# c0gent/hbbft

Hardware: AMD Instinct MI355X
Metric: verified BLS sig shares/sec (whole node) + combine latency, N=64 f=21 (higher is better)
Workload: dtype u32 limbs (Fp, 14x28-bit); 1 GPU; ThresholdSign share verification, BASELINE configs[1]; batch_per_gpu=65536, streams=2, documents_per_gpu=1024, n_nodes=64, f=21, pairing_impl=auto, parallelism=shard-by-batch x1

## Files before the change

hbbft_amd/csrc/ofp.hpp:

```cpp
#pragma once
#include "qfp.hpp"

namespace hbs {

HP_D int o_idx() { return (int)((threadIdx.x >> 1) & 3); }

HP_D int32_t o_swz4(int32_t v) { return __builtin_amdgcn_ds_swizzle(v, 0x101F); }
HP_D Fp o_swz4_fp(const Fp& a) {
  Fp r;
#pragma unroll
  for (int i = 0; i < NL; i++) r.l[i] = o_swz4(a.l[i]);
  return r;
}

HP_D Fp o_sel(int o, const Fp& a0, const Fp& a1, const Fp& a2, const Fp& a3) {
  const bool b0 = (o & 1) != 0, b1 = (o & 2) != 0;
  Fp r;
#pragma unroll
  for (int i = 0; i < NL; i++) {
    const int32_t lo = b0 ? a1.l[i] : a0.l[i];
    const int32_t hi = b0 ? a3.l[i] : a2.l[i];
    r.l[i] = b1 ? hi : lo;
  }
  return r;
}

HP_D void o_gather(int o, const Fp& mine, Fp (&r)[4]) {
  const Fp m1 = dpp_fp<DPP_QSWAP>(mine);
  const bool b0 = (o & 1) != 0, b1 = (o & 2) != 0;
  Fp e, d;
#pragma unroll
  for (int i = 0; i < NL; i++) {
    e.l[i] = b0 ? m1.l[i] : mine.l[i];
    d.l[i] = b0 ? mine.l[i] : m1.l[i];
  }
  const Fp e2 = o_swz4_fp(e), d2 = o_swz4_fp(d);
#pragma unroll
  for (int i = 0; i < NL; i++) {
    r[0].l[i] = b1 ? e2.l[i] : e.l[i];
    r[1].l[i] = b1 ? d2.l[i] : d.l[i];
    r[2].l[i] = b1 ? e.l[i] : e2.l[i];
    r[3].l[i] = b1 ? d.l[i] : d2.l[i];
  }
}

HP_D void h_mul4(const Fp (&x)[4], const Fp (&y)[4], Fp (&r)[4]) {
  const int o = o_idx();
  o_gather(o, h_mul(o_sel(o, x[0], x[1], x[2], x[3]), o_sel(o, y[0], y[1], y[2], y[3])), r);
}
HP_D void h_sqr4(const Fp (&x)[4], Fp (&r)[4]) {
  const int o = o_idx();
  o_gather(o, h_sqr(o_sel(o, x[0], x[1], x[2], x[3])), r);
}
HP_D void fp_mul4(const Fp (&x)[4], const Fp (&y)[4], Fp (&r)[4]) {
  const int o = o_idx();
  o_gather(o, fp_mul(o_sel(o, x[0], x[1], x[2], x[3]), o_sel(o, y[0], y[1], y[2], y[3])), r);
}

HP_D void h6_mul_pair_o(const H6& a, const H6& b, const H6& c, const H6& d, H6& ab, H6& cd) {
  Fp r[4];
  {
    const Fp x[4] = {a.c1, a.c2, c.c1, c.c2}, y[4] = {b.c1, b.c2, d.c1, d.c2};
    h_mul4(x, y, r);
  }
  const Fp av1 = r[0], av2 = r[1], cv1 = r[2], cv2 = r[3];
  {
    const Fp x[4] = {fp_addl(a.c1, a.c2), a.c0, fp_addl(c.c1, c.c2), c.c0};
    const Fp y[4] = {fp_add(b.c1, b.c2), b.c0, fp_add(d.c1, d.c2), d.c0};
    h_mul4(x, y, r);
  }
  const Fp av0 = r[1], cv0 = r[3];
  ab.c0 = fp_red_l(h_add_xi_l(av0, fp_sub2l(r[0], av1, av2)));
  cd.c0 = fp_red_l(h_add_xi_l(cv0, fp_sub2l(r[2], cv1, cv2)));
  {
    const Fp x[4] = {fp_addl(a.c0, a.c1), fp_addl(a.c0, a.c2), fp_addl(c.c0, c.c1), fp_addl(c.c0, c.c2)};
    const Fp y[4] = {fp_add(b.c0, b.c1), fp_add(b.c0, b.c2), fp_add(d.c0, d.c1), fp_add(d.c0, d.c2)};
    h_mul4(x, y, r);
  }
  ab.c1 = fp_red_l(h_add_xi_l(fp_sub2l(r[0], av0, av1), av2));
  ab.c2 = fp_red_l(fp_addl(fp_sub2l(r[1], av0, av2), av1));
  cd.c1 = fp_red_l(h_add_xi_l(fp_sub2l(r[2], cv0, cv1), cv2));
  cd.c2 = fp_red_l(fp_addl(fp_sub2l(r[3], cv0, cv2), cv1));
}

HP_D H6 h6_mul_o(const H6& a, const H6& b) {
  Fp r[4];
  {
    const Fp x[4] = {a.c1, a.c2, fp_addl(a.c1, a.c2), a.c0};
    const Fp y[4] = {b.c1, b.c2, fp_add(b.c1, b.c2), b.c0};
    h_mul4(x, y, r);
  }
  const Fp v1 = r[0], v2 = r[1], t12 = r[2], v0 = r[3];
  {
    const Fp x[4] = {fp_addl(a.c0, a.c1), fp_addl(a.c0, a.c2), a.c0, a.c0};
    const Fp y[4] = {fp_add(b.c0, b.c1), fp_add(b.c0, b.c2), b.c0, b.c0};
    h_mul4(x, y, r);
  }
  return {fp_red_l(h_add_xi_l(v0, fp_sub2l(t12, v1, v2))), fp_red_l(h_add_xi_l(fp_sub2l(r[0], v0, v1), v2)),
          fp_red_l(fp_addl(fp_sub2l(r[1], v0, v2), v1))};
}

HP_D H12 h12_cyclo_sqr_o(const H12& f) {
  const Fp& a0 = f.c0.c0; const Fp& a2 = f.c0.c1; const Fp& a4 = f.c0.c2;
  const Fp& a1 = f.c1.c0; const Fp& a3 = f.c1.c1; const Fp& a5 = f.c1.c2;
  Fp r1[4], r2[4];
  {
    const Fp x[4] = {a0, a3, a1, a4};
    h_sqr4(x, r1);
  }
  {
    const Fp x[4] = {fp_add(a0, a3), fp_add(a1, a4), a2, a5};
    h_sqr4(x, r2);
  }
  const Fp s25 = h_sqr(fp_add(a2, a5));
  const Fp &s0 = r1[0], &s3 = r1[1], &s1 = r1[2], &s4 = r1[3];
  const Fp &s03 = r2[0], &s14 = r2[1], &s2 = r2[2], &s5 = r2[3];
  H12 r;
  r.c0.c0 = fp_red_mk<3, -2>(h_add_xi_l(s0, s3), a0);
  r.c1.c1 = fp_red_mk<3, 2>(fp_sub2l(s03, s0, s3), a3);
  r.c0.c1 = fp_red_mk<3, -2>(h_add_xi_l(s1, s4), a2);
  r.c1.c2 = fp_red_mk<3, 2>(fp_sub2l(s14, s1, s4), a5);
  r.c0.c2 = fp_red_mk<3, -2>(h_add_xi_l(s2, s5), a4);
  r.c1.c0 = fp_red_mk<3, 2>(h_add_xi_l(fp_zero(), fp_sub2l(s25, s2, s5)), a1);
  return r;
}

HP_D H12 h12_frob1_o(const H12& f) {
  Fp r[4];
  const Fp x[4] = {h_conj(f.c1.c0), h_conj(f.c0.c1), h_conj(f.c1.c1), h_conj(f.c0.c2)};
  const Fp y[4] = {HP_FROB1(1), HP_FROB1(2), HP_FROB1(3), HP_FROB1(4)};
  h_mul4(x, y, r);
  H12 o;
  o.c0.c0 = h_conj(f.c0.c0);
  o.c1.c0 = r[0];
  o.c0.c1 = r[1];
  o.c1.c1 = r[2];
  o.c0.c2 = r[3];
  o.c1.c2 = h_mul(h_conj(f.c1.c2), HP_FROB1(5));
  return h12_red(o);
}
HP_D H12 h12_frob2_o(const H12& f) {
  Fp r[4];
  const Fp x[4] = {f.c1.c0, f.c0.c1, f.c1.c1, f.c0.c2};
  const Fp y[4] = {fp_const(hb::FROB2_1_C0), fp_const(hb::FROB2_2_C0), fp_const(hb::FROB2_3_C0),
                   fp_const(hb::FROB2_4_C0)};
  fp_mul4(x, y, r);
  H12 o;
  o.c0.c0 = f.c0.c0;
  o.c1.c0 = r[0];
  o.c0.c1 = r[1];
  o.c1.c1 = r[2];
  o.c0.c2 = r[3];
  o.c1.c2 = fp_mul(f.c1.c2, fp_const(hb::FROB2_5_C0));
  return o;
}

HP_D HLine h_dbl_step_o(HJac& T) {
  Fp r[4];
  {
    const Fp x[4] = {T.x, T.y, T.z, fp_add(T.y, T.z)};
    h_sqr4(x, r);
  }
  const Fp A = r[0], B = r[1], ZZ = r[2], YZ = r[3];
  const Fp E = fp_lin(3, A, 0, A);
  {
    const Fp xb = fp_add(T.x, B);
    const Fp x[4] = {B, xb, E, E}, y[4] = {B, xb, E, T.x};
    h_mul4(x, y, r);
  }
  const Fp C = r[0], XB = r[1], F = r[2], EX = r[3];
  const Fp D = fp_lin(2, fp_sub(fp_sub(XB, A), C), 0, C);
  const Fp Z3 = fp_sub(fp_sub(YZ, B), ZZ);
  const Fp X3 = fp_sub(F, fp_add(D, D));
  {
    const Fp x[4] = {E, Z3, E, E}, y[4] = {ZZ, ZZ, fp_sub(D, X3), ZZ};
    h_mul4(x, y, r);
  }
  HLine l;
  l.c0 = fp_reduce(fp_sub(EX, fp_add(B, B)));
  l.c1 = fp_neg(r[0]);
  l.c4 = r[1];
  T.y = fp_reduce(fp_sub(r[2], fp_lin(8, C, 0, C)));
  T.x = fp_reduce(X3);
  T.z = fp_reduce(Z3);
  return l;
}

HP_D HLine h_add_step_o(HJac& T, const Fp& xQ, const Fp& yQ) {
  Fp r[4];
  {
    const Fp x[4] = {T.z, yQ, T.z, T.z}, y[4] = {T.z, T.z, T.z, T.z};
    h_mul4(x, y, r);
  }
  const Fp Z1Z1 = r[0], YZ = r[1];
  {
    const Fp x[4] = {xQ, YZ, xQ, xQ}, y[4] = {Z1Z1, Z1Z1, Z1Z1, Z1Z1};
    h_mul4(x, y, r);
  }
  const Fp H = fp_sub(r[0], T.x);
  const Fp rr = fp_sub(r[1], T.y);
  {
    const Fp x[4] = {H, rr, T.z, H}, y[4] = {H, rr, H, H};
    h_mul4(x, y, r);
  }
  const Fp HH = r[0], R2 = r[1], Z3 = r[2];
  {
    const Fp x[4] = {H, T.x, yQ, rr}, y[4] = {HH, HH, Z3, xQ};
    h_mul4(x, y, r);
  }
  const Fp HHH = r[0], V = r[1], YZ3 = r[2], RX = r[3];
  const Fp X3 = fp_sub(fp_sub(R2, HHH), fp_add(V, V));
  {
    const Fp x[4] = {rr, T.y, rr, rr}, y[4] = {fp_sub(V, X3), HHH, fp_sub(V, X3), fp_sub(V, X3)};
    h_mul4(x, y, r);
  }
  HLine l;
  l.c0 = fp_reduce(fp_sub(RX, YZ3));
  l.c1 = fp_neg(rr);
  l.c4 = Z3;
  T.x = fp_reduce(X3);
  T.y = fp_reduce(fp_sub(r[0], r[1]));
  T.z = Z3;
  return l;
}

struct LaneOcto {
  static constexpr int LANES = 8;
  static HP_D bool leader() { return (threadIdx.x & 7) == 0; }
  static HP_D bool value_writer() { return o_idx() == 0; }
  using Walk = HJac;
  static HP_D HLine dbl_step(HJac& T) { return h_dbl_step_o(T); }
  static HP_D HLine add_step(HJac& T, const Fp& xQ, const Fp& yQ) { return h_add_step_o(T, xQ, yQ); }

  static HP_D H6 mul6(const H6& a, const H6& b) { return h6_mul_o(a, b); }
  template <class A1, class B1>
  static HP_D void mul6x2(const H6& a0, const H6& b0, const A1& a1, const B1& b1, H6& r0, H6& r1) {
    h6_mul_pair_o(a0, b0, h6_of(a1), h6_of(b1), r0, r1);
  }
  static HP_D void mul6x2_12(const H6& a0, const H6& b0, const H6& a1, const Fp& c1, const Fp& c2, H6& r0, H6& r1) {
    h6_mul_pair_o(a0, b0, a1, {h_zero(), c1, c2}, r0, r1);
  }
  static HP_D void line_product(const Fp& a0, const Fp& a1, const Fp& a4, const Fp& b0, const Fp& b1, const Fp& b4,
                                H6& C0, Fp& c11, Fp& c12) {
    Fp r[4];
    {
      const Fp x[4] = {a0, a1, a4, fp_addl(a0, a4)}, y[4] = {b0, b1, b4, fp_add(b0, b4)};
      h_mul4(x, y, r);
    }
    const Fp a0b0 = r[0], a1b1 = r[1], a4b4 = r[2], t04 = r[3];
    {
      const Fp x[4] = {fp_addl(a1, a4), fp_addl(a0, a1), a0, a0}, y[4] = {fp_add(b1, b4), fp_add(b0, b1), b0, b0};
      h_mul4(x, y, r);
    }
    h_line_comb(a0b0, a1b1, a4b4, t04, r[0], r[1], C0, c11, c12);
  }
  static HP_D H12 cyclo_sqr(const H12& f) { return h12_cyclo_sqr_o(f); }
  static HP_D H12 frob1(const H12& f) { return h12_frob1_o(f); }
  static HP_D H12 frob2(const H12& f) { return h12_frob2_o(f); }

  template <bool G1, bool G2, class RA, class RB, class ST>
  static HP_D void lines_at_p(const RA& raw_a, const RB& raw_b, const ST& A, const ST& B, bool neg2, HLine& la,
                              HLine& lb) {
    const HLine ra = raw_a();
    const HLine rb = raw_b();
    Fp r[4];
    const Fp x[4] = {ra.c1, ra.c4, rb.c1, rb.c4};
    const Fp y[4] = {side_xP<G1>(A), side_yP<G1>(A, false), side_xP<G2>(B), side_yP<G2>(B, neg2)};
    fp_mul4(x, y, r);
    la.c0 = A.act ? ra.c0 : h_one();
    la.c1 = A.act ? r[0] : fp_zero();
    la.c4 = A.act ? r[1] : fp_zero();
    lb.c0 = B.act ? rb.c0 : h_one();
    lb.c1 = B.act ? r[2] : fp_zero();
    lb.c4 = B.act ? r[3] : fp_zero();
  }
};

}
```

hbbft_amd/csrc/pair_side.hpp:

```cpp
#pragma once
#include "launch.hpp"
#include "qfp.hpp"

namespace hbs {

constexpr int PAIR_STEPS = 68;
constexpr int PL_Q4 = 11;
constexpr int STASH_WORDS = 72;

HP_D void stash_fp(uint32_t* __restrict__ s, const Fp& a) {
  const Fp r = fp_reduce(a);
  Fp rp = fp_addl(r, fp_const(P_L));
  fp_norm(rp);
  const Fp c = (r.l[NL - 1] < 0) ? rp : r;
#pragma unroll
  for (int w = 0; w < 12; w++) {
    const int bit = 32 * w, li = bit / 28, sh = bit % 28;
    uint64_t v = (uint64_t)(uint32_t)c.l[li] >> sh;
    if (li + 1 < NL) v |= (uint64_t)(uint32_t)c.l[li + 1] << (28 - sh);
    if (li + 2 < NL) v |= (uint64_t)(uint32_t)c.l[li + 2] << (56 - sh);
    s[w * 256] = (uint32_t)v;
  }
}
HP_D Fp unstash_fp(const uint32_t* __restrict__ s) {
  uint32_t w[12];
#pragma unroll
  for (int k = 0; k < 12; k++) w[k] = s[k * 256];
  Fp r;
#pragma unroll
  for (int i = 0; i < NL; i++) {
    const int bit = 28 * i, wi = bit >> 5, sh = bit & 31;
    uint64_t v = w[wi];
    if (wi + 1 < 12) v |= (uint64_t)w[wi + 1] << 32;
    r.l[i] = (int32_t)((uint32_t)(v >> sh) & (uint32_t)MASK28);
  }
  return r;
}
HP_D void stash12(uint32_t* __restrict__ s, const H12& f) {
  stash_fp(s + 0 * 12 * 256, f.c0.c0);
  stash_fp(s + 1 * 12 * 256, f.c0.c1);
  stash_fp(s + 2 * 12 * 256, f.c0.c2);
  stash_fp(s + 3 * 12 * 256, f.c1.c0);
  stash_fp(s + 4 * 12 * 256, f.c1.c1);
  stash_fp(s + 5 * 12 * 256, f.c1.c2);
}
HP_D H12 unstash12(const uint32_t* __restrict__ s) {
  H12 f;
  f.c0.c0 = unstash_fp(s + 0 * 12 * 256);
  f.c0.c1 = unstash_fp(s + 1 * 12 * 256);
  f.c0.c2 = unstash_fp(s + 2 * 12 * 256);
  f.c1.c0 = unstash_fp(s + 3 * 12 * 256);
  f.c1.c1 = unstash_fp(s + 4 * 12 * 256);
  f.c1.c2 = unstash_fp(s + 5 * 12 * 256);
  return f;
}

struct PairSide {
  const uint32_t* p;
  const uint32_t* q;
  const int4* lines;
  const uint8_t* qinf;
  const uint32_t* idx;
  uint32_t nq;
};

template <class ST>
HP_D void side_q(const PairSide& s, const ST& st, Fp& xQ, Fp& yQ) {
  h_g2_load(s.q + (size_t)st.q * 48, xQ, yQ);
  if (st.qinf) {
    xQ = h_one();
    yQ = h_one();
  }
}

template <bool WALK, bool GEN, class ST>
HP_D bool side_init(const PairSide& s, int i, bool negate, ST& st) {
  st.q = s.idx ? s.idx[i] : (uint32_t)i;
  if (st.q >= s.nq) return false;
  bool pinf;
  if (GEN) {
    pinf = false;
  } else if (s.p) {
    const uint32_t* w = s.p + (size_t)i * 24;
    pinf = words_zero(w, 24);
    st.xP = fp_from_words(w);
    st.yP = fp_from_words(w + 12);
  } else {
    pinf = false;
    st.xP = fp_const(hb::G1X_M);
    st.yP = fp_const(hb::G1Y_M);
  }
  if (!GEN && negate) st.yP = fp_neg(st.yP);
  if (WALK) {
    const uint32_t* w = s.q + (size_t)st.q * 48;
    st.qinf = lp_both(words_zero(w + (lp_even() ? 0 : 12), 12) && words_zero(w + (lp_even() ? 24 : 36), 12));
    Fp xQ, yQ;
    side_q(s, st, xQ, yQ);
    st.T = {xQ, yQ, h_one()};
  } else {
    st.qinf = s.qinf[st.q] != 0;
  }
  st.act = !pinf && !st.qinf;
  return true;
}

constexpr int LINE_Q4 = 2 * PL_Q4;
HP_D size_t line_at(size_t e) { return e * LINE_Q4 + (lp_even() ? 0 : PL_Q4); }
HP_D HLine line_load(const int4* __restrict__ p) {
  int32_t w[4 * PL_Q4];
#pragma unroll
  for (int k = 0; k < PL_Q4; k++) {
    const int4 v = p[k];
    w[4 * k] = v.x; w[4 * k + 1] = v.y; w[4 * k + 2] = v.z; w[4 * k + 3] = v.w;
  }
  HLine l;
#pragma unroll
  for (int j = 0; j < NL; j++) {
    l.c0.l[j] = w[j];
    l.c1.l[j] = w[NL + j];
    l.c4.l[j] = w[2 * NL + j];
  }
  return l;
}
HP_D void line_store(int4* __restrict__ p, const HLine& l) {
  int32_t w[4 * PL_Q4];
#pragma unroll
  for (int j = 0; j < NL; j++) {
    w[j] = l.c0.l[j];
    w[NL + j] = l.c1.l[j];
    w[2 * NL + j] = l.c4.l[j];
  }
  w[3 * NL] = 0;
  w[3 * NL + 1] = 0;
#pragma unroll
  for (int k = 0; k < PL_Q4; k++) p[k] = make_int4(w[4 * k], w[4 * k + 1], w[4 * k + 2], w[4 * k + 3]);
}

template <class G, bool WALK, bool DBL, class ST>
HP_D HLine side_raw(const PairSide& s, ST& st, int step) {
  if constexpr (!WALK) {
    return line_load(s.lines + line_at(st.q * PAIR_STEPS + step));
  } else if constexpr (DBL) {
    return G::dbl_step(st.T);
  } else {
    Fp xQ, yQ;
    side_q(s, st, xQ, yQ);
    return G::add_step(st.T, xQ, yQ);
  }
}

struct PairArgs {
  int n;
  PairSide s1, s2;
  int flags;
  uint8_t* verdict;
  uint32_t* value_out;
};


template <class G, bool PLUS1>
HP_D H12 exp_abs_x_gs(const H12& base) {
  const uint64_t e = PLUS1 ? hb::X_ABS + 1 : hb::X_ABS;
  H12 r = base;
#pragma unroll 1
  for (int k = 62; k >= 0; k--) {
    r = G::cyclo_sqr(r);
    if ((e >> k) & 1) r = h12_mul<G>(r, base);
  }
  return r;
}
template <class G>
struct ExpGs {
  HP_D H12 x(const H12& f) { return h12_conj(exp_abs_x_gs<G, false>(f)); }
  HP_D H12 xm1(const H12& f) { return h12_conj(exp_abs_x_gs<G, true>(f)); }
};

template <class G, class Exp>
HP_D H12 final_exp(const H12& f, uint32_t* __restrict__ stash) {
  const H12 f1 = h12_mul<G>(h12_conj(f), h12_inv<G>(f));
  const H12 g = h12_mul<G>(G::frob2(f1), f1);
  stash12(stash, g);
  Exp ex;
  H12 a = ex.xm1(ex.xm1(g));
  const H12 b = h12_mul<G>(ex.x(a), G::frob1(a));
  {
    const H12 gs = unstash12(stash);
    const H12 w = h12_mul<G>(h12_mul<G>(G::frob2(b), h12_conj(b)), h12_mul<G>(G::cyclo_sqr(gs), gs));
    stash12(stash, w);
  }
  const H12 c = ex.x(ex.x(b));
  return h12_mul<G>(c, unstash12(stash));
}

template <class G, class Exp, bool W1, bool W2, int GEN>
HP_D void lane_verify(const PairArgs& a, uint32_t* stash) {
  const int i = (int)((blockIdx.x * 256u + threadIdx.x) / (unsigned)G::LANES);
  if (i >= a.n) return;
  constexpr bool G1 = GEN == 1, G2 = GEN == 2;
  const bool neg2 = (a.flags & 1) != 0;
  SideStateT<typename G::Walk> A, B;
  const bool ok1 = side_init<W1, G1>(a.s1, i, false, A);
  const bool ok2 = side_init<W2, G2>(a.s2, i, neg2, B);
  if (!ok1 || !ok2) {
    if (G::leader() && a.verdict) a.verdict[i] = 0;
    return;
  }
  H12 f = h12_one();
  int step = 0;
#pragma unroll 1
  for (int b = 62; b >= 0; b--) {
    if (b != 62) f = h12_sqr<G>(f);
    {
      HLine la, lb;
      G::template lines_at_p<G1, G2>([&]() HP_L { return side_raw<G, W1, true>(a.s1, A, step); },
                                     [&]() HP_L { return side_raw<G, W2, true>(a.s2, B, step); }, A, B, neg2, la, lb);
      f = h12_mul_lines<G>(f, la.c0, la.c1, la.c4, lb.c0, lb.c1, lb.c4);
    }
    step++;
    if ((hb::X_ABS >> b) & 1) {
      HLine la, lb;
      G::template lines_at_p<G1, G2>([&]() HP_L { return side_raw<G, W1, false>(a.s1, A, step); },
                                     [&]() HP_L { return side_raw<G, W2, false>(a.s2, B, step); }, A, B, neg2, la, lb);
      f = h12_mul_lines<G>(f, la.c0, la.c1, la.c4, lb.c0, lb.c1, lb.c4);
      step++;
    }
  }
  if (a.flags & 2) f = h12_conj(f);
  const H12 e = final_exp<G, Exp>(f, stash + threadIdx.x);
  if (a.value_out && G::value_writer()) {
    uint32_t* o = a.value_out + (size_t)i * 144 + (lp_even() ? 0 : 12);
    fp_to_words(e.c0.c0, o + 0);
    fp_to_words(e.c0.c1, o + 24);
    fp_to_words(e.c0.c2, o + 48);
    fp_to_words(e.c1.c0, o + 72);
    fp_to_words(e.c1.c1, o + 96);
    fp_to_words(e.c1.c2, o + 120);
  }
  const bool one = h12_is_one(e);
  if (G::leader() && a.verdict) a.verdict[i] = one ? 1 : 0;
}

}

namespace hbl {

inline hbs::PairArgs pair_args(int n, const PairSideDesc& d1, const PairSideDesc& d2, int flags, uint8_t* verdict,
                               uint32_t* value_out) {
  hbs::PairArgs a;
  a.n = n;
  const PairSideDesc* d[2] = {&d1, &d2};
  hbs::PairSide* o[2] = {&a.s1, &a.s2};
  for (int k = 0; k < 2; k++) {
    o[k]->p = (const uint32_t*)d[k]->p;
    o[k]->q = (const uint32_t*)d[k]->q;
    o[k]->lines = (const int4*)d[k]->lines;
    o[k]->qinf = d[k]->qinf;
    o[k]->idx = d[k]->idx;
    o[k]->nq = (uint32_t)d[k]->nq;
  }
  a.flags = flags;
  a.verdict = verdict;
  a.value_out = value_out;
  return a;
}

inline int pair_gen_mode(const PairSideDesc& d1, const PairSideDesc& d2) {
  return (d1.p == nullptr) == (d2.p == nullptr) ? 0 : (d1.p == nullptr ? 1 : 2);
}

template <class K, int GEN>
hipError_t lane_launch(hipStream_t s, int n, const PairSideDesc& d1, const PairSideDesc& d2, int flags,
                       uint8_t* verdict, uint32_t* value_out) {
  const hbs::PairArgs a = pair_args(n, d1, d2, flags, verdict, value_out);
  const dim3 grid((unsigned)((K::LANES * (size_t)n + 255) / 256)), block(256);
  const size_t lds = (size_t)hbs::STASH_WORDS * 256 * 4;
  const bool w1 = d1.lines == nullptr, w2 = d2.lines == nullptr;
  if (w1 && w2)
    hipLaunchKernelGGL((K::template kernel<true, true, GEN>), grid, block, lds, s, a);
  else if (w1)
    hipLaunchKernelGGL((K::template kernel<true, false, GEN>), grid, block, lds, s, a);
  else if (w2)
    hipLaunchKernelGGL((K::template kernel<false, true, GEN>), grid, block, lds, s, a);
  else
    hipLaunchKernelGGL((K::template kernel<false, false, GEN>), grid, block, lds, s, a);
  return hipGetLastError();
}

}
```

hbbft_amd/csrc/pfp.hpp:

```cpp
#pragma once
#include "sfp.hpp"
#include "words.hpp"

#ifndef HP_INV_MODE
#define HP_INV_MODE 0
#endif

#define HP_D __device__ __forceinline__
#define HP_L __attribute__((always_inline))

namespace hbs {

constexpr int DPP_SWAP = 0xB1;
constexpr int DPP_EVEN = 0xA0;
constexpr int DPP_ODD = 0xF5;

HP_D bool lp_even() { return (threadIdx.x & 1) == 0; }
template <int CTRL>
HP_D int32_t dpp(int32_t v) {
  return __builtin_amdgcn_mov_dpp(v, CTRL, 0xF, 0xF, true);
}
template <int CTRL>
HP_D Fp dpp_fp(const Fp& a) {
  Fp r;
// ... 168 lines not shown
  const bool one = (ev ? part_one : mine_one) != 0;
  uint32_t v[N + 1];
#pragma unroll
  for (int i = 0; i <= N; i++) {
    const uint32_t pv = (uint32_t)dpp<DPP_SWAP>((int32_t)co[i]);
    v[i] = ev ? pv : co[i];
  }
  hb::words_reduce_32m<N>(v, mod);
#pragma unroll
  for (int i = 0; i < N; i++) out[i] = one ? v[i] : 0u;
}

template <int MODE = 0>
HP_D Fp h_inv_vartime(const Fp& a) {
  const Fp s = fp_sqr(a);
  const Fp n = fp_add(s, dpp_fp<DPP_SWAP>(s));
  uint32_t w[12], p[12], r[12];
  fp_to_words(n, w);
  uint32_t nz = 0;
#pragma unroll
  for (int i = 0; i < 12; i++) nz |= w[i];
  if (nz == 0) return fp_zero();
#pragma unroll
  for (int i = 0; i < 12; i++) p[i] = hb::PM2_W[i];
  p[0] += 2;
  if ((MODE & INV_PAIR) != 0)
    lp_inv_uniform<12>(w, p, r);
  else
    hb::words_inv_vartime<12, MODE>(w, p, r);
  return h_conj(fp_mul(a, fp_from_words(r)));
}

template <int M, int K>
HP_D Fp fp_red_mk(const Fp& t, const Fp& a) {
  const int64_t top = (int64_t)t.l[NL - 1] * M + (int64_t)K * a.l[NL - 1];
  const int32_t q = (int32_t)((top * QINV) >> 32);
  Fp r;
  int64_t acc = 0;
#pragma unroll
  for (int i = 0; i < NL - 1; i++) {
    acc += (int64_t)t.l[i] * M + (int64_t)K * a.l[i] - (int64_t)q * (int32_t)P_L[i];
    r.l[i] = (int32_t)acc & MASK28;
    acc >>= 28;
  }
  r.l[NL - 1] = (int32_t)(acc + top - (int64_t)q * (int32_t)P_L[NL - 1]);
  return r;
}
HP_D Fp fp_red_l(const Fp& t) { return fp_red_mk<1, 0>(t, t); }
HP_D Fp h_add_xi_l(const Fp& s, const Fp& t) {
  const int32_t sm = lp_even() ? -1 : 0;
  const Fp pt = dpp_fp<DPP_SWAP>(t);
  Fp r;
#pragma unroll
  for (int i = 0; i < NL; i++) r.l[i] = s.l[i] + t.l[i] + ((pt.l[i] ^ sm) - sm);
  return r;
}
HP_D Fp fp_sub2l(const Fp& a, const Fp& b, const Fp& c) {
  Fp r;
#pragma unroll
  for (int i = 0; i < NL; i++) r.l[i] = a.l[i] - b.l[i] - c.l[i];
  return r;
}

HP_D Fp h_xi_l(const Fp& t) {
  const int32_t sm = lp_even() ? -1 : 0;
  const Fp pt = dpp_fp<DPP_SWAP>(t);
  Fp r;
#pragma unroll
  for (int i = 0; i < NL; i++) r.l[i] = t.l[i] + ((pt.l[i] ^ sm) - sm);
  return r;
}

struct H6 { Fp c0, c1, c2; };
struct H12 { H6 c0, c1; };

HP_D H6 h6_zero() { return {h_zero(), h_zero(), h_zero()}; }
HP_D H6 h6_one() { return {h_one(), h_zero(), h_zero()}; }
HP_D H6 h6_add(const H6& a, const H6& b) { return {fp_add(a.c0, b.c0), fp_add(a.c1, b.c1), fp_add(a.c2, b.c2)}; }
HP_D H6 h6_sub(const H6& a, const H6& b) { return {fp_sub(a.c0, b.c0), fp_sub(a.c1, b.c1), fp_sub(a.c2, b.c2)}; }
HP_D H6 h6_neg(const H6& a) { return {fp_neg(a.c0), fp_neg(a.c1), fp_neg(a.c2)}; }
HP_D H6 h6_red(const H6& a) { return {fp_reduce(a.c0), fp_reduce(a.c1), fp_reduce(a.c2)}; }
HP_D H6 h6_mul_v(const H6& a) { return {h_mul_xi(a.c2), a.c0, a.c1}; }

HP_D H6 h6_mul(const H6& a, const H6& b) {
  const Fp v1 = h_mul(a.c1, b.c1);
  const Fp v2 = h_mul(a.c2, b.c2);
  const Fp d0 = fp_sub2l(h_mul(fp_addl(a.c1, a.c2), fp_add(b.c1, b.c2)), v1, v2);
  const Fp v0 = h_mul(a.c0, b.c0);
  const Fp c0 = fp_red_l(h_add_xi_l(v0, d0));
  const Fp c1 = fp_red_l(h_add_xi_l(fp_sub2l(h_mul(fp_addl(a.c0, a.c1), fp_add(b.c0, b.c1)), v0, v1), v2));
  const Fp c2 = fp_red_l(fp_addl(fp_sub2l(h_mul(fp_addl(a.c0, a.c2), fp_add(b.c0, b.c2)), v0, v2), v1));
  return {c0, c1, c2};
}
HP_D H6 h6_inv(const H6& a) {
  const Fp c0 = fp_reduce(fp_sub(h_sqr(a.c0), h_mul_xi(h_mul(a.c1, a.c2))));
  const Fp c1 = fp_reduce(fp_sub(h_mul_xi(h_sqr(a.c2)), h_mul(a.c0, a.c1)));
  const Fp c2 = fp_reduce(fp_sub(h_sqr(a.c1), h_mul(a.c0, a.c2)));
  const Fp t = fp_reduce(fp_add(h_mul(a.c0, c0), h_mul_xi(fp_add(h_mul(a.c2, c1), h_mul(a.c1, c2)))));
  const Fp ti = fp_reduce(h_inv_vartime<HP_INV_MODE>(t));
  return {h_mul(c0, ti), h_mul(c1, ti), h_mul(c2, ti)};
}

HP_D H12 h12_one() { return {h6_one(), h6_zero()}; }
HP_D H12 h12_conj(const H12& a) { return {a.c0, h6_neg(a.c1)}; }
HP_D H12 h12_red(const H12& a) { return {h6_red(a.c0), h6_red(a.c1)}; }
HP_D H12 h12_kcomb(const H6& t0, const H6& t1, const H6& s) {
  return {{fp_red_l(h_add_xi_l(t0.c0, t1.c2)), fp_red_l(fp_addl(t0.c1, t1.c0)), fp_red_l(fp_addl(t0.c2, t1.c1))},
          {fp_red_l(fp_sub2l(s.c0, t0.c0, t1.c0)), fp_red_l(fp_sub2l(s.c1, t0.c1, t1.c1)),
           fp_red_l(fp_sub2l(s.c2, t0.c2, t1.c2))}};
}

HP_D H6 h6_mul_12(const H6& x, const Fp& b1, const Fp& b2) {
  const Fp u = h_mul(x.c1, b1);
  const Fp w = h_mul(x.c2, b2);
  const Fp c0 = fp_red_l(h_xi_l(fp_sub2l(h_mul(fp_addl(x.c1, x.c2), fp_add(b1, b2)), u, w)));
  const Fp c1 = fp_red_l(h_add_xi_l(h_mul(x.c0, b1), w));
  const Fp c2 = fp_red_l(fp_addl(h_mul(x.c0, b2), u));
  return {c0, c1, c2};
}

HP_D const H6& h6_of(const H6& a) { return a; }
template <class F>
HP_D auto h6_of(const F& f) -> decltype(f()) { return f(); }

template <class G>
HP_D H12 h12_mul(const H12& a, const H12& b) {
  H6 t0, t1;
  G::mul6x2(a.c0, b.c0, a.c1, b.c1, t0, t1);
  const H6 s = G::mul6(h6_add(a.c0, a.c1), h6_add(b.c0, b.c1));
  return h12_kcomb(t0, t1, s);
}
template <class G>
HP_D H12 h12_sqr(const H12& a) {
  H6 t, s;
  G::mul6x2(a.c0, a.c1, [&]() HP_L { return h6_add(a.c0, a.c1); },
            [&]() HP_L { return h6_red(h6_add(a.c0, h6_mul_v(a.c1))); }, t, s);
  return {{fp_red_l(h_add_xi_l(fp_subl(s.c0, t.c0), fp_subl(fp_zero(), t.c2))), fp_red_l(fp_sub2l(s.c1, t.c1, t.c0)),
           fp_red_l(fp_sub2l(s.c2, t.c2, t.c1))},
          {fp_red_l(fp_addl(t.c0, t.c0)), fp_red_l(fp_addl(t.c1, t.c1)), fp_red_l(fp_addl(t.c2, t.c2))}};
}
template <class G>
HP_D H12 h12_mul_lines(const H12& f, const Fp& a0, const Fp& a1, const Fp& a4, const Fp& b0, const Fp& b1,
                       const Fp& b4) {
  H6 C0, t0, t1;
  Fp c11, c12;
  G::line_product(a0, a1, a4, b0, b1, b4, C0, c11, c12);
  G::mul6x2_12(f.c0, C0, f.c1, c11, c12, t0, t1);
  const H6 s = G::mul6(h6_add(f.c0, f.c1), {C0.c0, fp_add(C0.c1, c11), fp_add(C0.c2, c12)});
  return h12_kcomb(t0, t1, s);
}
template <class G>
HP_D H12 h12_inv(const H12& a) {
  H6 s0, s1, r0, r1;
  G::mul6x2(a.c0, a.c0, a.c1, a.c1, s0, s1);
  const H6 t = h6_red(h6_sub(h6_red(s0), h6_red(h6_mul_v(h6_red(s1)))));
  const H6 ti = h6_red(h6_inv(t));
  G::mul6x2(a.c0, ti, a.c1, ti, r0, r1);
  return h12_red({r0, h6_neg(r1)});
}

#define HP_FROB1(K) h_const(hb::FROB1_##K##_C0, hb::FROB1_##K##_C1)
HP_D H12 h12_frob1(const H12& f) {
  H12 r;
  r.c0.c0 = h_conj(f.c0.c0);
  r.c1.c0 = h_mul(h_conj(f.c1.c0), HP_FROB1(1));
  r.c0.c1 = h_mul(h_conj(f.c0.c1), HP_FROB1(2));
  r.c1.c1 = h_mul(h_conj(f.c1.c1), HP_FROB1(3));
  r.c0.c2 = h_mul(h_conj(f.c0.c2), HP_FROB1(4));
  r.c1.c2 = h_mul(h_conj(f.c1.c2), HP_FROB1(5));
  return h12_red(r);
}
HP_D H12 h12_frob2(const H12& f) {
  H12 r;
  r.c0.c0 = f.c0.c0;
  r.c1.c0 = fp_mul(f.c1.c0, fp_const(hb::FROB2_1_C0));
  r.c0.c1 = fp_mul(f.c0.c1, fp_const(hb::FROB2_2_C0));
  r.c1.c1 = fp_mul(f.c1.c1, fp_const(hb::FROB2_3_C0));
  r.c0.c2 = fp_mul(f.c0.c2, fp_const(hb::FROB2_4_C0));
  r.c1.c2 = fp_mul(f.c1.c2, fp_const(hb::FROB2_5_C0));
  return r;
}

HP_D H12 h12_cyclo_sqr(const H12& f) {
  const Fp& a0 = f.c0.c0; const Fp& a2 = f.c0.c1; const Fp& a4 = f.c0.c2;
  const Fp& a1 = f.c1.c0; const Fp& a3 = f.c1.c1; const Fp& a5 = f.c1.c2;
  H12 r;
  {
    const Fp s0 = h_sqr(a0), s3 = h_sqr(a3), s03 = h_sqr(fp_add(a0, a3));
    r.c0.c0 = fp_red_mk<3, -2>(h_add_xi_l(s0, s3), a0);
    r.c1.c1 = fp_red_mk<3, 2>(fp_sub2l(s03, s0, s3), a3);
  }
  {
    const Fp s1 = h_sqr(a1), s4 = h_sqr(a4), s14 = h_sqr(fp_add(a1, a4));
    r.c0.c1 = fp_red_mk<3, -2>(h_add_xi_l(s1, s4), a2);
    r.c1.c2 = fp_red_mk<3, 2>(fp_sub2l(s14, s1, s4), a5);
  }
  {
    const Fp s2 = h_sqr(a2), s5 = h_sqr(a5), s25 = h_sqr(fp_add(a2, a5));
    r.c0.c2 = fp_red_mk<3, -2>(h_add_xi_l(s2, s5), a4);
    r.c1.c0 = fp_red_mk<3, 2>(h_add_xi_l(fp_zero(), fp_sub2l(s25, s2, s5)), a1);
  }
  return r;
}

struct HC { Fp a1, a2, a4, a5; };

HP_D HC hc_compress(const H12& f) { return {f.c1.c0, f.c0.c1, f.c0.c2, f.c1.c2}; }
HP_D HC hc_sqr(const HC& c) {
  HC r;
  {
    const Fp s1 = h_sqr(c.a1), s4 = h_sqr(c.a4), s14 = h_sqr(fp_add(c.a1, c.a4));
    r.a2 = fp_red_mk<3, -2>(h_add_xi_l(s1, s4), c.a2);
    r.a5 = fp_red_mk<3, 2>(fp_sub2l(s14, s1, s4), c.a5);
  }
  {
    const Fp s2 = h_sqr(c.a2), s5 = h_sqr(c.a5), s25 = h_sqr(fp_add(c.a2, c.a5));
    r.a4 = fp_red_mk<3, -2>(h_add_xi_l(s2, s5), c.a4);
    r.a1 = fp_red_mk<3, 2>(h_add_xi_l(fp_zero(), fp_sub2l(s25, s2, s5)), c.a1);
  }
  return r;
}
HP_D Fp hc_denom(const Fp& a1) { return fp_lin(4, a1, 0, a1); }
HP_D H12 hc_decompress(const HC& c, const Fp& di) {
  const Fp s5 = h_sqr(c.a5), s2 = h_sqr(c.a2);
  Fp t = h_xi_l(s5);
#pragma unroll
  for (int i = 0; i < NL; i++) t.l[i] += 3 * s2.l[i];
  const Fp a3 = h_mul(fp_red_mk<1, -2>(t, c.a4), di);
  const Fp u = fp_addl(fp_lin(2, h_sqr(a3), -3, h_mul(c.a4, c.a2)), h_mul(c.a1, c.a5));
  const Fp a0 = fp_red_l(h_add_xi_l(h_one(), u));
  return {{a0, c.a2, c.a4}, {c.a1, a3, c.a5}};
}

HP_D bool h12_is_one(const H12& f) {
  bool ok = fp_is_zero(fp_sub(f.c0.c0, h_one()));
  ok = ok && fp_is_zero(f.c0.c1) && fp_is_zero(f.c0.c2);
  ok = ok && fp_is_zero(f.c1.c0) && fp_is_zero(f.c1.c1) && fp_is_zero(f.c1.c2);
  return lp_both(ok);
}

struct HJac { Fp x, y, z; };
struct HLine { Fp c0, c1, c4; };

struct HProj { Fp x, y, z; };

HP_D HLine h_dbl_step_h(HProj& T) {
  const Fp C = h_sqr(T.z);
  const Fp YZ = h_sqr(fp_add(T.y, T.z));
  const Fp B = h_sqr(T.y);
  const Fp H = fp_sub(fp_sub(YZ, B), C);
  const Fp E = fp_red_mk<12, 0>(h_xi_l(C), C);
  const Fp A = h_mul(T.x, T.y);
  const Fp S = h_sqr(T.x);
  HLine l;
  l.c0 = fp_red_mk<1, -1>(B, E);
  l.c1 = fp_lin(-3, S, 0, S);
  l.c4 = H;
  const Fp Bm = fp_lin(1, B, -3, E);
  const Fp Bp = fp_lin(1, B, 3, E);
  T.x = h_mul(fp_addl(A, A), Bm);
  const Fp EE = h_sqr(E);
  T.y = fp_red_mk<1, -12>(h_sqr(Bp), EE);
  const Fp BH = h_mul(fp_addl(B, B), H);
  T.z = fp_red_mk<2, 0>(BH, BH);
  return l;
}

HP_D HLine h_add_step_h(HProj& T, const Fp& xQ, const Fp& yQ) {
  const Fp th = fp_sub(T.y, h_mul(yQ, T.z));
  const Fp la = fp_sub(T.x, h_mul(xQ, T.z));
  HLine l;
  l.c0 = fp_reduce(fp_sub(h_mul(th, xQ), h_mul(la, yQ)));
  l.c1 = fp_neg(th);
  l.c4 = la;
  const Fp C = h_sqr(th);
  const Fp D = h_sqr(la);
  const Fp E = h_mul(la, D);
  const Fp F = h_mul(T.z, C);
  const Fp G = h_mul(T.x, D);
  const Fp H = fp_lin(1, fp_addl(E, F), -2, G);
  const Fp X3 = h_mul(la, H);
  T.y = fp_reduce(fp_sub(h_mul(th, fp_sub(G, H)), h_mul(E, T.y)));
  T.z = h_mul(T.z, E);
  T.x = X3;
  return l;
}

template <class PT>
struct SideStateT {
  Fp xP, yP;
  bool act;
  bool qinf;
  uint32_t q;
  PT T;
};

template <bool GEN, class ST>
HP_D Fp side_xP(const ST& st) { return GEN ? fp_const(hb::G1X_M) : st.xP; }
template <bool GEN, class ST>
HP_D Fp side_yP(const ST& st, bool negate) {
  return GEN ? (negate ? fp_neg(fp_const(hb::G1Y_M)) : fp_const(hb::G1Y_M)) : st.yP;
}

struct LanePair {
  static constexpr int LANES = 2;
  static HP_D bool leader() { return lp_even(); }
  static HP_D bool value_writer() { return true; }
  using Walk = HProj;
  static HP_D HLine dbl_step(HProj& T) { return h_dbl_step_h(T); }
  static HP_D HLine add_step(HProj& T, const Fp& xQ, const Fp& yQ) { return h_add_step_h(T, xQ, yQ); }

  static HP_D H6 mul6(const H6& a, const H6& b) { return h6_mul(a, b); }
  template <class A1, class B1>
  static HP_D void mul6x2(const H6& a0, const H6& b0, const A1& a1, const B1& b1, H6& r0, H6& r1) {
    r0 = h6_mul(a0, b0);
    r1 = h6_mul(h6_of(a1), h6_of(b1));
  }
  static HP_D void mul6x2_12(const H6& a0, const H6& b0, const H6& a1, const Fp& c1, const Fp& c2, H6& r0, H6& r1) {
    r0 = h6_mul(a0, b0);
    r1 = h6_mul_12(a1, c1, c2);
  }
  static HP_D void line_product(const Fp& a0, const Fp& a1, const Fp& a4, const Fp& b0, const Fp& b1, const Fp& b4,
                                H6& C0, Fp& c11, Fp& c12) {
    const Fp a0b0 = h_mul(a0, b0);
    const Fp a1b1 = h_mul(a1, b1);
    const Fp a4b4 = h_mul(a4, b4);
    c11 = fp_red_l(fp_sub2l(h_mul(fp_addl(a0, a4), fp_add(b0, b4)), a0b0, a4b4));
    c12 = fp_red_l(fp_sub2l(h_mul(fp_addl(a1, a4), fp_add(b1, b4)), a1b1, a4b4));
    C0 = {fp_red_l(h_add_xi_l(a0b0, a4b4)), fp_red_l(fp_sub2l(h_mul(fp_addl(a0, a1), fp_add(b0, b1)), a0b0, a1b1)),
          a1b1};
  }
  static HP_D H12 cyclo_sqr(const H12& f) { return h12_cyclo_sqr(f); }
  static HP_D H12 frob1(const H12& f) { return h12_frob1(f); }
  static HP_D H12 frob2(const H12& f) { return h12_frob2(f); }

  template <bool GEN, class ST>
  static HP_D HLine line_at_p(const HLine& l, const ST& st, bool negate) {
    HLine e;
    e.c0 = st.act ? l.c0 : h_one();
    e.c1 = st.act ? fp_mul(l.c1, side_xP<GEN>(st)) : fp_zero();
    e.c4 = st.act ? fp_mul(l.c4, side_yP<GEN>(st, negate)) : fp_zero();
    return e;
  }
  template <bool G1, bool G2, class RA, class RB, class ST>
  static HP_D void lines_at_p(const RA& raw_a, const RB& raw_b, const ST& A, const ST& B, bool neg2, HLine& la,
                              HLine& lb) {
    la = line_at_p<G1>(raw_a(), A, false);
    lb = line_at_p<G2>(raw_b(), B, neg2);
  }
};

HP_D void h_g2_load(const uint32_t* __restrict__ w, Fp& x, Fp& y) {
  const int o = lp_even() ? 0 : 12;
  x = fp_from_words(w + o);
  y = fp_from_words(w + 24 + o);
}
HP_D bool words_zero(const uint32_t* __restrict__ w, int n) {
  uint32_t o = 0;
  for (int k = 0; k < n; k++) o |= w[k];
  return o == 0;
}

}
```

hbbft_amd/csrc/qfp.hpp:

```cpp
#pragma once
#include "pfp.hpp"

namespace hbs {

constexpr int DPP_QSWAP = 0x4E;

HP_D bool q_hi() { return (threadIdx.x & 2) != 0; }

HP_D Fp q_sel(bool hi, const Fp& a, const Fp& b) {
  Fp r;
#pragma unroll
  for (int i = 0; i < NL; i++) r.l[i] = hi ? b.l[i] : a.l[i];
  return r;
}
HP_D H6 q_sel6(bool hi, const H6& a, const H6& b) { return {q_sel(hi, a.c0, b.c0), q_sel(hi, a.c1, b.c1), q_sel(hi, a.c2, b.c2)}; }

HP_D void q_join(bool hi, const Fp& mine, Fp& v0, Fp& v1) {
  const Fp o = dpp_fp<DPP_QSWAP>(mine);
  v0 = q_sel(hi, mine, o);
  v1 = q_sel(hi, o, mine);
}
HP_D void q_join6(bool hi, const H6& mine, H6& v0, H6& v1) {
  q_join(hi, mine.c0, v0.c0, v1.c0);
  q_join(hi, mine.c1, v0.c1, v1.c1);
  q_join(hi, mine.c2, v0.c2, v1.c2);
}

HP_D void h_mul2(const Fp& x0, const Fp& y0, const Fp& x1, const Fp& y1, Fp& r0, Fp& r1) {
  const bool hi = q_hi();
  q_join(hi, h_mul(q_sel(hi, x0, x1), q_sel(hi, y0, y1)), r0, r1);
}
HP_D void h_sqr2(const Fp& a0, const Fp& a1, Fp& r0, Fp& r1) {
  const bool hi = q_hi();
  q_join(hi, h_sqr(q_sel(hi, a0, a1)), r0, r1);
}
HP_D void fp_mul2(const Fp& x0, const Fp& y0, const Fp& x1, const Fp& y1, Fp& r0, Fp& r1) {
  const bool hi = q_hi();
  q_join(hi, fp_mul(q_sel(hi, x0, x1), q_sel(hi, y0, y1)), r0, r1);
}
HP_D void h6_mul2(const H6& a0, const H6& b0, const H6& a1, const H6& b1, H6& r0, H6& r1) {
  const bool hi = q_hi();
  q_join6(hi, h6_mul(q_sel6(hi, a0, a1), q_sel6(hi, b0, b1)), r0, r1);
}

HP_D H6 h6_mul_q(const H6& a, const H6& b) {
  Fp v1, v2, t12, v0, t01, t02;
  h_mul2(a.c1, b.c1, a.c2, b.c2, v1, v2);
  h_mul2(fp_addl(a.c1, a.c2), fp_add(b.c1, b.c2), a.c0, b.c0, t12, v0);
  const Fp c0 = fp_red_l(h_add_xi_l(v0, fp_sub2l(t12, v1, v2)));
  h_mul2(fp_addl(a.c0, a.c1), fp_add(b.c0, b.c1), fp_addl(a.c0, a.c2), fp_add(b.c0, b.c2), t01, t02);
  const Fp c1 = fp_red_l(h_add_xi_l(fp_sub2l(t01, v0, v1), v2));
  const Fp c2 = fp_red_l(fp_addl(fp_sub2l(t02, v0, v2), v1));
  return {c0, c1, c2};
}

HP_D void h_line_comb(const Fp& a0b0, const Fp& a1b1, const Fp& a4b4, const Fp& t04, const Fp& t14, const Fp& t01,
                      H6& C0, Fp& c11, Fp& c12) {
  c11 = fp_red_l(fp_sub2l(t04, a0b0, a4b4));
  c12 = fp_red_l(fp_sub2l(t14, a1b1, a4b4));
  C0 = {fp_red_l(h_add_xi_l(a0b0, a4b4)), fp_red_l(fp_sub2l(t01, a0b0, a1b1)), a1b1};
}

HP_D H12 h12_cyclo_sqr_q(const H12& f) {
  const Fp& a0 = f.c0.c0; const Fp& a2 = f.c0.c1; const Fp& a4 = f.c0.c2;
  const Fp& a1 = f.c1.c0; const Fp& a3 = f.c1.c1; const Fp& a5 = f.c1.c2;
  Fp s0, s3, s03, s1, s4, s14, s2, s5;
  h_sqr2(a0, a3, s0, s3);
  h_sqr2(fp_add(a0, a3), a1, s03, s1);
  h_sqr2(a4, fp_add(a1, a4), s4, s14);
  h_sqr2(a2, a5, s2, s5);
  const Fp s25 = h_sqr(fp_add(a2, a5));
  H12 r;
  r.c0.c0 = fp_red_mk<3, -2>(h_add_xi_l(s0, s3), a0);
  r.c1.c1 = fp_red_mk<3, 2>(fp_sub2l(s03, s0, s3), a3);
  r.c0.c1 = fp_red_mk<3, -2>(h_add_xi_l(s1, s4), a2);
  r.c1.c2 = fp_red_mk<3, 2>(fp_sub2l(s14, s1, s4), a5);
  r.c0.c2 = fp_red_mk<3, -2>(h_add_xi_l(s2, s5), a4);
  r.c1.c0 = fp_red_mk<3, 2>(h_add_xi_l(fp_zero(), fp_sub2l(s25, s2, s5)), a1);
  return r;
}

HP_D H12 h12_frob1_q(const H12& f) {
  H12 r;
  r.c0.c0 = h_conj(f.c0.c0);
  h_mul2(h_conj(f.c1.c0), HP_FROB1(1), h_conj(f.c0.c1), HP_FROB1(2), r.c1.c0, r.c0.c1);
  h_mul2(h_conj(f.c1.c1), HP_FROB1(3), h_conj(f.c0.c2), HP_FROB1(4), r.c1.c1, r.c0.c2);
  r.c1.c2 = h_mul(h_conj(f.c1.c2), HP_FROB1(5));
  return h12_red(r);
}
HP_D H12 h12_frob2_q(const H12& f) {
  H12 r;
  r.c0.c0 = f.c0.c0;
  fp_mul2(f.c1.c0, fp_const(hb::FROB2_1_C0), f.c0.c1, fp_const(hb::FROB2_2_C0), r.c1.c0, r.c0.c1);
  fp_mul2(f.c1.c1, fp_const(hb::FROB2_3_C0), f.c0.c2, fp_const(hb::FROB2_4_C0), r.c1.c1, r.c0.c2);
  r.c1.c2 = fp_mul(f.c1.c2, fp_const(hb::FROB2_5_C0));
  return r;
}

HP_D HLine h_dbl_step_q(HJac& T) {
  Fp A, B, C, ZZ, XB, YZ, EX, EZ, C4, F;
  h_sqr2(T.x, T.y, A, B);
  h_sqr2(B, T.z, C, ZZ);
  h_sqr2(fp_add(T.x, B), fp_add(T.y, T.z), XB, YZ);
  const Fp D = fp_lin(2, fp_sub(fp_sub(XB, A), C), 0, C);
  const Fp E = fp_lin(3, A, 0, A);
  h_mul2(E, T.x, E, ZZ, EX, EZ);
  HLine l;
  l.c0 = fp_sub(EX, fp_add(B, B));
  l.c1 = fp_neg(EZ);
  const Fp Z3 = fp_sub(fp_sub(YZ, B), ZZ);
  h_mul2(Z3, ZZ, E, E, C4, F);
  l.c4 = C4;
  const Fp X3 = fp_sub(F, fp_add(D, D));
  T.y = fp_sub(h_mul(E, fp_sub(D, X3)), fp_lin(8, C, 0, C));
  T.x = X3;
  T.z = Z3;
  l.c0 = fp_reduce(l.c0);
  T.x = fp_reduce(T.x);
  T.y = fp_reduce(T.y);
  T.z = fp_reduce(T.z);
  return l;
}

HP_D HLine h_add_step_q(HJac& T, const Fp& xQ, const Fp& yQ) {
  Fp YZ, U2, S2, Z3, HH, R2, HHH, V, RV, YH, RX, YZ3;
  const Fp Z1Z1 = h_sqr(T.z);
  h_mul2(yQ, T.z, xQ, Z1Z1, YZ, U2);
  const Fp H = fp_sub(U2, T.x);
  h_mul2(YZ, Z1Z1, T.z, H, S2, Z3);
  const Fp r = fp_sub(S2, T.y);
  h_sqr2(H, r, HH, R2);
  h_mul2(H, HH, T.x, HH, HHH, V);
  const Fp X3 = fp_sub(fp_sub(R2, HHH), fp_add(V, V));
  h_mul2(r, fp_sub(V, X3), T.y, HHH, RV, YH);
  h_mul2(r, xQ, yQ, Z3, RX, YZ3);
  HLine l;
  l.c0 = fp_reduce(fp_sub(RX, YZ3));
  l.c1 = fp_neg(r);
  l.c4 = Z3;
  T.x = fp_reduce(X3);
  T.y = fp_reduce(fp_sub(RV, YH));
  T.z = Z3;
  return l;
}

struct LaneQuad {
  static constexpr int LANES = 4;
  static HP_D bool leader() { return (threadIdx.x & 3) == 0; }
  static HP_D bool value_writer() { return !q_hi(); }
  using Walk = HJac;
  static HP_D HLine dbl_step(HJac& T) { return h_dbl_step_q(T); }
  static HP_D HLine add_step(HJac& T, const Fp& xQ, const Fp& yQ) { return h_add_step_q(T, xQ, yQ); }

  static HP_D H6 mul6(const H6& a, const H6& b) { return h6_mul_q(a, b); }
  template <class A1, class B1>
  static HP_D void mul6x2(const H6& a0, const H6& b0, const A1& a1, const B1& b1, H6& r0, H6& r1) {
    h6_mul2(a0, b0, h6_of(a1), h6_of(b1), r0, r1);
  }
  static HP_D void mul6x2_12(const H6& a0, const H6& b0, const H6& a1, const Fp& c1, const Fp& c2, H6& r0, H6& r1) {
    h6_mul2(a0, b0, a1, {h_zero(), c1, c2}, r0, r1);
  }
  static HP_D void line_product(const Fp& a0, const Fp& a1, const Fp& a4, const Fp& b0, const Fp& b1, const Fp& b4,
                                H6& C0, Fp& c11, Fp& c12) {
    Fp a0b0, a1b1, a4b4, t04, t14, t01;
    h_mul2(a0, b0, a1, b1, a0b0, a1b1);
    h_mul2(a4, b4, fp_addl(a0, a4), fp_add(b0, b4), a4b4, t04);
    h_mul2(fp_addl(a1, a4), fp_add(b1, b4), fp_addl(a0, a1), fp_add(b0, b1), t14, t01);
    h_line_comb(a0b0, a1b1, a4b4, t04, t14, t01, C0, c11, c12);
  }
  static HP_D H12 cyclo_sqr(const H12& f) { return h12_cyclo_sqr_q(f); }
  static HP_D H12 frob1(const H12& f) { return h12_frob1_q(f); }
  static HP_D H12 frob2(const H12& f) { return h12_frob2_q(f); }

  template <bool GEN, class ST>
  static HP_D HLine line_at_p(const HLine& l, const ST& st, bool negate) {
    HLine e;
    e.c0 = st.act ? l.c0 : h_one();
    Fp c1, c4;
    fp_mul2(l.c1, side_xP<GEN>(st), l.c4, side_yP<GEN>(st, negate), c1, c4);
    e.c1 = st.act ? c1 : fp_zero();
    e.c4 = st.act ? c4 : fp_zero();
    return e;
  }
  template <bool G1, bool G2, class RA, class RB, class ST>
  static HP_D void lines_at_p(const RA& raw_a, const RB& raw_b, const ST& A, const ST& B, bool neg2, HLine& la,
                              HLine& lb) {
    la = line_at_p<G1>(raw_a(), A, false);
    lb = line_at_p<G2>(raw_b(), B, neg2);
  }
};

}
```

Measured before the change: 3.680 million shares/s.

## Park Miller-loop walk point and P coordinates in LDS stash for LanePair

For the two-lane pairing path, the Miller loop's running G2 point T and the G1 coordinates xP/yP are now kept in the per-thread LDS stash columns between steps. They are reloaded only when a doubling or addition step or a line evaluation needs them. The loop also evaluates the walking side first when only side B walks. The aim is to lower register pressure in the Miller loop so occupancy rises or spills drop, at the cost of extra volatile LDS traffic on every step.

```diff
diff --git a/hbbft_amd/csrc/ofp.hpp b/hbbft_amd/csrc/ofp.hpp
--- a/hbbft_amd/csrc/ofp.hpp
+++ b/hbbft_amd/csrc/ofp.hpp
@@ -229,6 +229,8 @@
   static HP_D bool leader() { return (threadIdx.x & 7) == 0; }
   static HP_D bool value_writer() { return o_idx() == 0; }
   using Walk = HJac;
+  template <bool W1, bool W2, int GEN>
+  using Park = NoPark;
   static HP_D HLine dbl_step(HJac& T) { return h_dbl_step_o(T); }
   static HP_D HLine add_step(HJac& T, const Fp& xQ, const Fp& yQ) { return h_add_step_o(T, xQ, yQ); }
 
@@ -258,9 +260,9 @@
   static HP_D H12 frob1(const H12& f) { return h12_frob1_o(f); }
   static HP_D H12 frob2(const H12& f) { return h12_frob2_o(f); }
 
-  template <bool G1, bool G2, class RA, class RB, class ST>
+  template <bool G1, bool G2, bool WALK_FIRST, class RA, class RB, class ST>
   static HP_D void lines_at_p(const RA& raw_a, const RB& raw_b, const ST& A, const ST& B, bool neg2, HLine& la,
-                              HLine& lb) {
+                              HLine& lb, const NoPark&) {
     const HLine ra = raw_a();
     const HLine rb = raw_b();
     Fp r[4];
diff --git a/hbbft_amd/csrc/pair_side.hpp b/hbbft_amd/csrc/pair_side.hpp
--- a/hbbft_amd/csrc/pair_side.hpp
+++ b/hbbft_amd/csrc/pair_side.hpp
@@ -7,6 +7,7 @@
 constexpr int PAIR_STEPS = 68;
 constexpr int PL_Q4 = 11;
 constexpr int STASH_WORDS = 72;
+static_assert(PARK_WORDS <= STASH_WORDS, "the Miller loop parks T and P in the stash (pfp.hpp PairPark)");
 
 HP_D void stash_fp(uint32_t* __restrict__ s, const Fp& a) {
   const Fp r = fp_reduce(a);
@@ -136,16 +137,16 @@
   for (int k = 0; k < PL_Q4; k++) p[k] = make_int4(w[4 * k], w[4 * k + 1], w[4 * k + 2], w[4 * k + 3]);
 }
 
-template <class G, bool WALK, bool DBL, class ST>
-HP_D HLine side_raw(const PairSide& s, ST& st, int step) {
+template <class G, bool WALK, bool DBL, int SIDE, class ST, class PK>
+HP_D HLine side_raw(const PairSide& s, ST& st, int step, const PK& pk) {
   if constexpr (!WALK) {
     return line_load(s.lines + line_at(st.q * PAIR_STEPS + step));
   } else if constexpr (DBL) {
-    return G::dbl_step(st.T);
+    return pk.template walk<SIDE>(st, [&](typename G::Walk& T) HP_L { return G::dbl_step(T); });
   } else {
     Fp xQ, yQ;
     side_q(s, st, xQ, yQ);
-    return G::add_step(st.T, xQ, yQ);
+    return pk.template walk<SIDE>(st, [&](typename G::Walk& T) HP_L { return G::add_step(T, xQ, yQ); });
   }
 }
 
@@ -205,6 +206,9 @@
     if (G::leader() && a.verdict) a.verdict[i] = 0;
     return;
   }
+  const typename G::template Park<W1, W2, GEN> pk(stash + threadIdx.x);
+  pk.init(A, B);
+  constexpr bool WF = !W1 && W2;
   H12 f = h12_one();
   int step = 0;
 #pragma unroll 1
@@ -212,15 +216,17 @@
     if (b != 62) f = h12_sqr<G>(f);
     {
       HLine la, lb;
-      G::template lines_at_p<G1, G2>([&]() HP_L { return side_raw<G, W1, true>(a.s1, A, step); },
-                                     [&]() HP_L { return side_raw<G, W2, true>(a.s2, B, step); }, A, B, neg2, la, lb);
+      G::template lines_at_p<G1, G2, WF>([&]() HP_L { return side_raw<G, W1, true, 0>(a.s1, A, step, pk); },
+                                         [&]() HP_L { return side_raw<G, W2, true, 1>(a.s2, B, step, pk); }, A, B, neg2,
+                                         la, lb, pk);
       f = h12_mul_lines<G>(f, la.c0, la.c1, la.c4, lb.c0, lb.c1, lb.c4);
     }
     step++;
     if ((hb::X_ABS >> b) & 1) {
       HLine la, lb;
-      G::template lines_at_p<G1, G2>([&]() HP_L { return side_raw<G, W1, false>(a.s1, A, step); },
-                                     [&]() HP_L { return side_raw<G, W2, false>(a.s2, B, step); }, A, B, neg2, la, lb);
+      G::template lines_at_p<G1, G2, WF>([&]() HP_L { return side_raw<G, W1, false, 0>(a.s1, A, step, pk); },
+                                         [&]() HP_L { return side_raw<G, W2, false, 1>(a.s2, B, step, pk); }, A, B, neg2,
+                                         la, lb, pk);
       f = h12_mul_lines<G>(f, la.c0, la.c1, la.c4, lb.c0, lb.c1, lb.c4);
       step++;
     }
diff --git a/hbbft_amd/csrc/pfp.hpp b/hbbft_amd/csrc/pfp.hpp
--- a/hbbft_amd/csrc/pfp.hpp
+++ b/hbbft_amd/csrc/pfp.hpp
@@ -494,6 +494,101 @@
   return GEN ? (negate ? fp_neg(fp_const(hb::G1Y_M)) : fp_const(hb::G1Y_M)) : st.yP;
 }
 
+struct NoPark {
+  HP_D explicit NoPark(uint32_t*) {}
+  template <class ST>
+  HP_D void init(const ST&, const ST&) const {}
+  template <int SIDE, class ST, class F>
+  HP_D HLine walk(ST& st, const F& f) const { return f(st.T); }
+  template <int SIDE, class ST>
+  HP_D Fp xP(const ST& st) const { return st.xP; }
+  template <int SIDE, class ST>
+  HP_D Fp yP(const ST& st) const { return st.yP; }
+};
+
+constexpr int PARK_WORDS = 72;
+constexpr int park_fit(int used, bool need, int words) { return need && used + words <= PARK_WORDS ? used : -1; }
+typedef volatile __attribute__((address_space(3))) uint32_t* ParkCol;
+
+HP_D void park_put(ParkCol c, int slot, const Fp& a) {
+#pragma unroll
+  for (int i = 0; i < NL; i++) c[(slot + i) * 256] = (uint32_t)a.l[i];
+}
+HP_D Fp park_get(ParkCol c, int slot) {
+  Fp r;
+#pragma unroll
+  for (int i = 0; i < NL; i++) r.l[i] = (int32_t)c[(slot + i) * 256];
+  return r;
+}
+
+template <bool W1, bool W2, int GEN>
+struct PairPark {
+  static constexpr int TW = 3 * NL, PW = 2 * NL;
+  static constexpr int T_B = park_fit(0, W2, TW);
+  static constexpr int U1 = T_B < 0 ? 0 : TW;
+  static constexpr int T_A = park_fit(U1, W1, TW);
+  static constexpr int U2 = U1 + (T_A < 0 ? 0 : TW);
+  static constexpr int P_A = park_fit(U2, GEN != 1, PW);
+  static constexpr int U3 = U2 + (P_A < 0 ? 0 : PW);
+  static constexpr int P_B = park_fit(U3, GEN != 2, PW);
+  template <int SIDE>
+  static constexpr int t_slot() { return SIDE == 0 ? T_A : T_B; }
+  template <int SIDE>
+  static constexpr int p_slot() { return SIDE == 0 ? P_A : P_B; }
+
+  ParkCol col;
+  HP_D explicit PairPark(uint32_t* c) : col((ParkCol)c) {}
+
+  template <int SIDE>
+  HP_D void put_T(const HProj& T) const {
+    park_put(col, t_slot<SIDE>(), T.x);
+    park_put(col, t_slot<SIDE>() + NL, T.y);
+    park_put(col, t_slot<SIDE>() + 2 * NL, T.z);
+  }
+  template <int SIDE, class ST>
+  HP_D void init_side(const ST& st) const {
+    if constexpr (t_slot<SIDE>() >= 0) put_T<SIDE>(st.T);
+    if constexpr (p_slot<SIDE>() >= 0) {
+      park_put(col, p_slot<SIDE>(), st.xP);
+      park_put(col, p_slot<SIDE>() + NL, st.yP);
+    }
+  }
+  template <class ST>
+  HP_D void init(const ST& A, const ST& B) const {
+    init_side<0>(A);
+    init_side<1>(B);
+  }
+  template <int SIDE, class ST, class F>
+  HP_D HLine walk(ST& st, const F& f) const {
+    if constexpr (t_slot<SIDE>() < 0) {
+      return f(st.T);
+    } else {
+      HProj T;
+      T.z = park_get(col, t_slot<SIDE>() + 2 * NL);
+      T.y = park_get(col, t_slot<SIDE>() + NL);
+      T.x = park_get(col, t_slot<SIDE>());
+      const HLine l = f(T);
+      put_T<SIDE>(T);
+      return l;
+    }
+  }
+  template <int SIDE, class ST>
+  HP_D Fp xP(const ST& st) const {
+    if constexpr (p_slot<SIDE>() < 0) return st.xP; else return park_get(col, p_slot<SIDE>());
+  }
+  template <int SIDE, class ST>
+  HP_D Fp yP(const ST& st) const {
+    if constexpr (p_slot<SIDE>() < 0) return st.yP; else return park_get(col, p_slot<SIDE>() + NL);
+  }
+};
+
+#ifndef HP_PARK
+#define HP_PARK 1
+#endif
+#ifndef HP_WALK_FIRST
+#define HP_WALK_FIRST 1
+#endif
+
 struct LanePair {
   static constexpr int LANES = 2;
   static HP_D bool leader() { return lp_even(); }
@@ -526,19 +621,34 @@
   static HP_D H12 frob1(const H12& f) { return h12_frob1(f); }
   static HP_D H12 frob2(const H12& f) { return h12_frob2(f); }
 
-  template <bool GEN, class ST>
-  static HP_D HLine line_at_p(const HLine& l, const ST& st, bool negate) {
+#if HP_PARK
+  template <bool W1, bool W2, int GEN>
+  using Park = PairPark<W1, W2, GEN>;
+#else
+  template <bool W1, bool W2, int GEN>
+  using Park = NoPark;
+#endif
+
+  template <bool GEN, int SIDE, class ST, class PK>
+  static HP_D HLine line_at_p(const HLine& l, const ST& st, bool negate, const PK& pk) {
     HLine e;
     e.c0 = st.act ? l.c0 : h_one();
-    e.c1 = st.act ? fp_mul(l.c1, side_xP<GEN>(st)) : fp_zero();
-    e.c4 = st.act ? fp_mul(l.c4, side_yP<GEN>(st, negate)) : fp_zero();
+    const Fp c1 = fp_mul(l.c1, GEN ? side_xP<true>(st) : pk.template xP<SIDE>(st));
+    e.c1 = st.act ? c1 : fp_zero();
+    const Fp c4 = fp_mul(l.c4, GEN ? side_yP<true>(st, negate) : pk.template yP<SIDE>(st));
+    e.c4 = st.act ? c4 : fp_zero();
     return e;
   }
-  template <bool G1, bool G2, class RA, class RB, class ST>
+  template <bool G1, bool G2, bool WALK_FIRST, class RA, class RB, class ST, class PK>
   static HP_D void lines_at_p(const RA& raw_a, const RB& raw_b, const ST& A, const ST& B, bool neg2, HLine& la,
-                              HLine& lb) {
-    la = line_at_p<G1>(raw_a(), A, false);
-    lb = line_at_p<G2>(raw_b(), B, neg2);
+                              HLine& lb, const PK& pk) {
+    if constexpr (WALK_FIRST && HP_WALK_FIRST) {
+      lb = line_at_p<G2, 1>(raw_b(), B, neg2, pk);
+      la = line_at_p<G1, 0>(raw_a(), A, false, pk);
+    } else {
+      la = line_at_p<G1, 0>(raw_a(), A, false, pk);
+      lb = line_at_p<G2, 1>(raw_b(), B, neg2, pk);
+    }
   }
 };
 
diff --git a/hbbft_amd/csrc/qfp.hpp b/hbbft_amd/csrc/qfp.hpp
--- a/hbbft_amd/csrc/qfp.hpp
+++ b/hbbft_amd/csrc/qfp.hpp
@@ -149,6 +149,8 @@
   static HP_D bool leader() { return (threadIdx.x & 3) == 0; }
   static HP_D bool value_writer() { return !q_hi(); }
   using Walk = HJac;
+  template <bool W1, bool W2, int GEN>
+  using Park = NoPark;
   static HP_D HLine dbl_step(HJac& T) { return h_dbl_step_q(T); }
   static HP_D HLine add_step(HJac& T, const Fp& xQ, const Fp& yQ) { return h_add_step_q(T, xQ, yQ); }
 
@@ -182,9 +184,9 @@
     e.c4 = st.act ? c4 : fp_zero();
     return e;
   }
-  template <bool G1, bool G2, class RA, class RB, class ST>
+  template <bool G1, bool G2, bool WALK_FIRST, class RA, class RB, class ST>
   static HP_D void lines_at_p(const RA& raw_a, const RB& raw_b, const ST& A, const ST& B, bool neg2, HLine& la,
-                              HLine& lb) {
+                              HLine& lb, const NoPark&) {
     la = line_at_p<G1>(raw_a(), A, false);
     lb = line_at_p<G2>(raw_b(), B, neg2);
   }
```

Result: faster. 3.790 million shares/s, median of 6 (+3.0%).
